# ai4colonoscopy/PraNet-V2

Measured on AMD Instinct MI355X. Metric: images/sec (train fwd+bwd) at 352x352 bs=32/GPU, higher is better.
Workload: dtype bf16; 1 GPU; PraNet-V2 Res2Net50 training step (fwd+4x structure_loss+bwd+clamp+Adam), bs=32/GPU 352x352, random-init, synthetic ellipse masks; global_batch=32, parallelism=dp1, launch=hipGraph replay

## Files before the change

include/pn2.h:

```cpp
#ifndef PN2_H
#define PN2_H
#ifdef __cplusplus
extern "C" {
#endif

#define PN2_F32 0
#define PN2_BF16 1
#define PN2_F32F 2
#define PN2_F32X3 3
#define PN2_CONV_STATS 1
#define PN2_CONV_ACCUM 2
#define PN2_CONV_SPLITK(n) ((n) << 16)
#define PN2_CONV_ROWGATE 8
#define PN2_CONV_AFFINE 16
#define PN2_CONV_RELU 32
#define PN2_CONV_RELU6 64
#define PN2_CONV_BIAS 4

typedef struct pn2_conv_desc {
    int N, H, W;
    int OH, OW;
    int Cin_p, ld_in;
    int Cout, ld_out;
    int KH, KW, stride, pad_h, pad_w, dil_h, dil_w;
// ... 26 lines not shown
int pn2_conv_stat_blocks(int m, int cout, int dtype);
int pn2_conv_gemm(int dtype, const void* in, const void* wp, void* out, float* psum, float* psq, const pn2_conv_desc* d, void* stream);
#define PN2_BNB_STATS 1
#define PN2_BNB_MASK_RAW 2
#define PN2_BNB_MASK_Y 4
#define PN2_BNB_STORE_MASKED 8
int pn2_conv_gemm_gated(int dtype, const void* in, const void* wp, void* out, float* psum, float* psq, const pn2_conv_desc* d, const float* gate, void* stream);
int pn2_conv_gemm_affine(int dtype, const void* in, const void* wp, void* out, const float* scale, const float* shift, const void* res, int ld_res,
                         const pn2_conv_desc* d, void* stream);
typedef struct pn2_bnb_target {
    void* out; int ld_out;
    int mode;
    const void* raw; int ld_raw;
    const void* y; int ld_y;
    const float* par; int ps;
    int split;
    const void* raw2; const float* par2;
    float* p1; float* p2; int ldp;
} pn2_bnb_target;
typedef struct pn2_conv_ep { pn2_bnb_target a, b; const void* pool; int ld_pool; int pad_; pn2_bnb_target c; } pn2_conv_ep;
int pn2_conv_gemm_ep(int dtype, const void* in, const void* wp, void* out, const pn2_conv_desc* d, const pn2_conv_ep* ep, void* stream);
typedef struct pn2_conv_job { const void* in; const void* wp; void* out; float* psum; float* psq; pn2_conv_desc d; int pad_; pn2_conv_ep ep; } pn2_conv_job;
int pn2_conv_gemm_tile(int dtype, const pn2_conv_desc* d);
int pn2_conv_gemm_job_blocks(int dtype, const pn2_conv_job* j, int bm, int bn);
int pn2_conv_gemm_multi(int dtype, int bm, int bn, int ep, const pn2_conv_job* jobs_dev, const int* block_start_dev, int njobs, int total_blocks, void* stream);
int pn2_conv_splitk_reduce(int dtype, const float* ws, int ksplit, int M, int Cout, void* out, int ld_out, const float* bias, float* psum, float* psq,
                           int accumulate, void* stream);
int pn2_conv_wgrad(int dtype, const void* dy, const void* x, float* slab, const pn2_wgrad_desc* d, int nsplit, void* stream);
typedef struct pn2_wgrad_job { const void* dy; const void* x; float* slab; pn2_wgrad_desc d; int nsplit;
    int rot;
} pn2_wgrad_job;
int pn2_conv_wgrad_variant(int dtype, const pn2_wgrad_desc* d);
int pn2_conv_wgrad_blocks(const pn2_wgrad_desc* d, int nsplit);
int pn2_conv_wgrad_multi(int dtype, int variant, const pn2_wgrad_job* jobs_dev, const int* block_start_dev, int njobs, int total_blocks, void* stream);
int pn2_pack_weight(int dtype, const float* w_oihw, void* wp, const pn2_pack_desc* p, void* stream);
int pn2_wgrad_reduce(const float* slab, float* gw_oihw, const pn2_pack_desc* p, int nsplit, int accumulate, void* stream);
int pn2_pack_patch_weight(int dtype, const float* w_oihw, void* wp, int Cout, int Cin, int KH, int KW, int Cin_p, int Rp, int Kp, void* stream);
int pn2_depth_to_space(int dtype, const void* t, int ld_t, void* dx, int ld_dx, int N, int H, int W, int OH, int OW, int S, int C, int accumulate, void* stream);
int pn2_conv_dgrad_small_cin(int dtype, const void* dy, int ld_dy, const float* w_oihw, void* dx, int ld_dx, int N, int H, int W, int OH, int OW,
                             int Cout, int Cin, int KH, int KW, int stride, int pad, int accumulate, void* stream);
typedef struct pn2_pack_job { const float* w; void* wp; pn2_pack_desc d; } pn2_pack_job;
int pn2_pack_blocks(const pn2_pack_desc* p);
int pn2_pack_weights_multi(int dtype, const pn2_pack_job* jobs_dev, const int* block_start_dev, int njobs, int total_blocks, void* stream);
typedef struct pn2_reduce_job { const float* slab; float* gw; pn2_pack_desc d; int nsplit; int accumulate; } pn2_reduce_job;
int pn2_wgrad_reduce_blocks(const pn2_pack_desc* p);
int pn2_wgrad_reduce_multi(const pn2_reduce_job* jobs_dev, const int* block_start_dev, int njobs, int total_blocks, void* stream);

typedef struct pn2_bn_desc {
    int M;
    int Cp;
    int C, gw, gwp;
    float eps, momentum;
    int ldp;
    int tile_rows;
} pn2_bn_desc;
int pn2_bn_finalize(const float* psum, const float* psq, int nblk, const pn2_bn_desc* d, const float* gamma, const float* beta,
                    float* running_mean, float* running_var, float* scale, float* shift, float* mean, float* invstd, void* stream);
int pn2_bn_eval_prepare(const pn2_bn_desc* d, const float* gamma, const float* beta, const float* running_mean, const float* running_var,
                        float* scale, float* shift, void* stream);
typedef struct pn2_bnprep_job { const float* gamma; const float* beta; const float* running_mean; const float* running_var; float* scale; float* shift; pn2_bn_desc d; int pad_; } pn2_bnprep_job;
int pn2_bn_eval_prepare_multi(const pn2_bnprep_job* jobs_dev, const int* block_start_dev, int njobs, int total_blocks, void* stream);
int pn2_affine_act(int dt_in, const void* x, int ld_x, int dt_out, void* y, int ld_y, int M, int Cout,
                   const float* scale, const float* shift, const void* res, int ld_res, int relu, void* stream);
int pn2_affine_act_sum(int dt, const void* x, int ld_x, void* y, int ld_y, int M, int C, const float* scale, const float* shift, int relu,
                       const void* add, int ld_add, void* y2, int ld_y2, void* stream);
int pn2_affine_act_tee(int dt, const void* x, int ld_x, void* y, int ld_y, int M, int C, const float* scale, const float* shift, int relu,
// ... 289 lines not shown
```

pranet-v2_amd/csrc/pn2_conv.hip:

```cpp
#include <cstring>
#include "pn2_common.h"
#include "../../include/pn2.h"

namespace {

constexpr int ROWB = 128;
constexpr int KSUB = ROWB / 64;
constexpr int RS = ROWB;

#ifdef PN2_STAMP
constexpr int PN2_STAMP_SLOTS = 16, PN2_STAMP_BLOCKS = 1 << 16;
__device__ unsigned long long pn2_stamp_buf[PN2_STAMP_BLOCKS * PN2_STAMP_SLOTS];
__device__ __forceinline__ void pn2_stamp(int i) {
    if (threadIdx.x == 0 && blockIdx.y == 0 && blockIdx.x < PN2_STAMP_BLOCKS) pn2_stamp_buf[blockIdx.x * PN2_STAMP_SLOTS + i] = __builtin_amdgcn_s_memtime();
}
__device__ __forceinline__ void pn2_stamp_hw() {
    if (threadIdx.x == 0 && blockIdx.y == 0 && blockIdx.x < PN2_STAMP_BLOCKS) {
        pn2_stamp_buf[blockIdx.x * PN2_STAMP_SLOTS + 10] = __builtin_amdgcn_s_getreg((31 << 11) | 4);
        pn2_stamp_buf[blockIdx.x * PN2_STAMP_SLOTS + 11] = __builtin_amdgcn_s_getreg((31 << 11) | 20);
    }
}
#define PN2_STAMP_AT(i) pn2_stamp(i)
#else
#define PN2_STAMP_AT(i)
// ... 1694 lines not shown
#pragma unroll
                for (int i = 0; i < MT; ++i) {
                    asm volatile("ds_read_b64_tr_b16 %0, %1" : "=v"(a0[i]) : "v"(sb + offA[i] + ks * 32 * RBY));
                    asm volatile("ds_read_b64_tr_b16 %0, %1" : "=v"(a1[i]) : "v"(sb + offA[i] + (ks * 32 + 16) * RBY));
                }
#pragma unroll
                for (int j = 0; j < NT; ++j) {
                    asm volatile("ds_read_b64_tr_b16 %0, %1" : "=v"(b0[j]) : "v"(sb + offB[j] + ks * 32 * RBX));
                    asm volatile("ds_read_b64_tr_b16 %0, %1" : "=v"(b1[j]) : "v"(sb + offB[j] + (ks * 32 + 16) * RBX));
                }
                asm volatile("s_waitcnt lgkmcnt(0)" ::: "memory");
                __builtin_amdgcn_sched_barrier(0);
#pragma unroll
                for (int i = 0; i < MT; ++i)
#pragma unroll
                    for (int j = 0; j < NT; ++j)
                        MMA<bf16_t>::run(acc[i][j], make_uint4(a0[i].x, a0[i].y, a1[i].x, a1[i].y), make_uint4(b0[j].x, b0[j].y, b1[j].x, b1[j].y));
            }
        }
    }
#undef PN2_WISSUE
    float* dst = slab + ((size_t)split * d.Rp + co0) * d.Kp + k0;
#pragma unroll
    for (int i = 0; i < MT; ++i)
#pragma unroll
        for (int j = 0; j < NT; ++j) {
            if (BNK > 128 && k0 + wn * WTN + j * 16 >= d.Kp) continue;
#pragma unroll
            for (int r = 0; r < 4; ++r)
                dst[(size_t)(wm * WTM + i * 16 + g * 4 + r) * d.Kp + wn * WTN + j * 16 + l15] = acc[i][j][r];
        }
}

template <typename T, int BMC, int BNK, int WM, int WN, bool PW>
__global__ __launch_bounds__(256) void conv_wgrad(const T* __restrict__ dy, const T* __restrict__ x, float* __restrict__ slab, pn2_wgrad_desc d, int nsplit) {
    conv_wgrad_body<T, BMC, BNK, WM, WN, PW>(dy, x, slab, d, nsplit, blockIdx.x);
}
template <typename T, int BMC, int BNK, int WM, int WN, bool PW>
__global__ __launch_bounds__(256) void conv_wgrad_tab(const pn2_wgrad_job* __restrict__ jobs, const int* __restrict__ bstart, int njobs) {
    const int total = bstart[njobs];
    for (int b = blockIdx.x; b < total; b += gridDim.x) {
        const int jb = find_job(bstart, njobs, b);
        const pn2_wgrad_job j = jobs[jb];
        const int bl = b - bstart[jb];
        conv_wgrad_body<T, BMC, BNK, WM, WN, PW>((const T*)j.dy, (const T*)j.x, j.slab, j.d, j.nsplit, (bl & ~7) | ((bl - j.rot) & 7));
        __syncthreads();
    }
}
template <int BMC, int WM, int WN, bool PW, int BNK = 128>
__global__ __launch_bounds__(256) void conv_wgrad_dma(const bf16_t* __restrict__ dy, const bf16_t* __restrict__ x, float* __restrict__ slab, pn2_wgrad_desc d, int nsplit) {
    conv_wgrad_dma_body<BMC, WM, WN, PW, BNK>(dy, x, slab, d, nsplit, blockIdx.x);
}
template <int BMC, int WM, int WN, bool PW, int BNK = 128>
__global__ __launch_bounds__(256) void conv_wgrad_dma_tab(const pn2_wgrad_job* __restrict__ jobs, const int* __restrict__ bstart, int njobs) {
    const int total = bstart[njobs];
    for (int b = blockIdx.x; b < total; b += gridDim.x) {
        const int jb = find_job(bstart, njobs, b);
        const pn2_wgrad_job j = jobs[jb];
        const int bl = b - bstart[jb];
        conv_wgrad_dma_body<BMC, WM, WN, PW, BNK>((const bf16_t*)j.dy, (const bf16_t*)j.x, j.slab, j.d, j.nsplit, (bl & ~7) | ((bl - j.rot) & 7));
        __syncthreads();
    }
}

template <int BMC, int WM, int WN, int BNK>
__global__ __launch_bounds__(256, 2) void conv_wgrad_dma_tab_mix(const pn2_wgrad_job* __restrict__ jobs, const int* __restrict__ bstart, int njobs) {
    const int total = bstart[njobs];
    for (int b = blockIdx.x; b < total; b += gridDim.x) {
        const int jb = find_job(bstart, njobs, b);
        const pn2_wgrad_job j = jobs[jb];
        const int bl = b - bstart[jb];
        const int lb = (bl & ~7) | ((bl - j.rot) & 7);
        if (j.d.KH == 1 && j.d.KW == 1 && j.d.stride == 1 && j.d.pad_h == 0 && j.d.pad_w == 0)
            conv_wgrad_dma_body<BMC, WM, WN, true, BNK>((const bf16_t*)j.dy, (const bf16_t*)j.x, j.slab, j.d, j.nsplit, lb);
        else
            conv_wgrad_dma_body<BMC, WM, WN, false, BNK>((const bf16_t*)j.dy, (const bf16_t*)j.x, j.slab, j.d, j.nsplit, lb);
        __syncthreads();
// ... 324 lines not shown
}
template <bool EP>
int gemm_multi_dispatch(int dtype, int bm, int bn, int bits, const pn2_conv_job* jobs, const int* bstart, int njobs, int total, hipStream_t st) {
    const bool ks2 = dtype == PN2_BF16 && (bm & TILE_KS2);
    if (ks2) bm &= 0xff;
    return with_dtype(dtype, [&](auto ty) {
        using T = typename decltype(ty)::type;
        return with_tile(bm, bn, [&](auto tile) {
            using L = decltype(tile);
            constexpr int BM = L::BM, BN = L::BN, WM = L::WM, WN = L::WN;
            if constexpr (sizeof(T) == 2) {
                if constexpr (BN >= 64 && !(BM == 128 && BN == 128)) { if (ks2) return launch_dma_tab_ks2<EP, BM, BN, WM, WN>(jobs, bstart, njobs, total, bits, st); }
                else if (ks2) return -2;
                return launch_dma_tab<EP, BM, BN, WM, WN>(jobs, bstart, njobs, total, bits, st);
            } else if constexpr (BN == 128) return -2;
            else return launch_gather_tab_f32<T, EP, BM, BN, WM, WN>(jobs, bstart, njobs, total, st);
        });
    });
}

constexpr int wg_dma_ring_bytes(int bmc, int bnk) { return 3 * wg_px(bmc) * (bmc * 2 + bnk * 2); }

template <int BMC, int WM, int WN, int BNK = 128>
int launch_wgrad_dma(const void* dy, const void* x, float* slab, const pn2_wgrad_desc& d, int nsplit, hipStream_t st) {
    constexpr int PX = wg_px(BMC), max_b = wg_dma_ring_bytes(BMC, BNK);
    const int M = d.N * d.OH * d.OW;
    const int total_steps = (M + PX - 1) / PX, spb = (total_steps + nsplit - 1) / nsplit;
    const int lds = (spb < 3 ? (spb < 1 ? 1 : spb) : 3) * (max_b / 3);
    const dim3 grid(8 * ((nsplit + 7) / 8) * (d.Rp / BMC) * ((d.Kp + BNK - 1) / BNK));
    if (is_pointwise(d)) return pn2_launch<conv_wgrad_dma<BMC, WM, WN, true, BNK>>(grid, dim3(256), lds, max_b, st, (const bf16_t*)dy, (const bf16_t*)x, slab, d, nsplit);
    return pn2_launch<conv_wgrad_dma<BMC, WM, WN, false, BNK>>(grid, dim3(256), lds, max_b, st, (const bf16_t*)dy, (const bf16_t*)x, slab, d, nsplit);
}

template <typename T>
int wgrad_variant(const pn2_wgrad_desc& d) {
    const int bmc = pn2_wgrad_tile_co(d.Cout_p);
    bool dma = false, wide = false;
    if constexpr (sizeof(T) == 2) {
        dma = d.tune ? d.tune >= 2 : (is_pointwise(d) && d.N * d.OH * d.OW >= 8192);
        if ((size_t)d.N * d.OH * d.OW * d.ld_dy * 2 >= 0x80000000ull || (size_t)d.N * d.H * d.W * d.ld_x * 2 >= 0x80000000ull) dma = false;
        wide = dma && bmc == 128 && d.Kp >= 256 && d.tune == 3;
    }
    if (wide) return 12 + (is_pointwise(d) ? 1 : 0);
    return (dma ? 6 : 0) + (bmc == 128 ? 2 : (bmc == 64 ? 1 : 0)) * 2 + (is_pointwise(d) ? 1 : 0);
}

template <typename T>
inline int wgrad_blocks_t(const pn2_wgrad_desc& d, int nsplit) {
    const int bmc = pn2_wgrad_tile_co(d.Cout_p);
    const int bnk = wgrad_variant<T>(d) >= 12 ? 256 : 128;
    return 8 * ((nsplit + 7) / 8) * (d.Rp / bmc) * ((d.Kp + bnk - 1) / bnk);
}

template <typename T>
int wgrad_dispatch(const void* dy, const void* x, float* slab, const pn2_wgrad_desc& d, int nsplit, hipStream_t st) {
    const int bmc = pn2_wgrad_tile_co(d.Cout_p);
    if (d.Rp % bmc || d.Kp % 128) return -2;
    const int v = wgrad_variant<T>(d);
    return with_wgrad_tile(bmc, [&](auto tile) {
        using L = decltype(tile);
        if constexpr (sizeof(T) == 2) {
            if (v >= 12) return launch_wgrad_dma<128, 2, 2, 256>(dy, x, slab, d, nsplit, st);
            if (v >= 6) return launch_wgrad_dma<L::BM, L::WM, L::WN>(dy, x, slab, d, nsplit, st);
        }
        return launch_wgrad<T, L::BM, L::WM, L::WN>(dy, x, slab, d, nsplit, st);
    });
}

template <typename T, int BMC, int WM, int WN>
int launch_wgrad_tab(bool pw, const pn2_wgrad_job* jobs, const int* bstart, int njobs, int total, hipStream_t st) {
    constexpr int BNK = 128;
    constexpr int lds = 2 * wg_stage_bytes<T>(BMC, BNK), cap = X3<T> ? lds : 0;
    if (pw) return pn2_launch<conv_wgrad_tab<T, BMC, BNK, WM, WN, true>>(dim3(total), dim3(256), lds, cap, st, jobs, bstart, njobs);
    return pn2_launch<conv_wgrad_tab<T, BMC, BNK, WM, WN, false>>(dim3(total), dim3(256), lds, cap, st, jobs, bstart, njobs);
}

template <int BMC, int WM, int WN, int BNK = 128>
int launch_wgrad_dma_tab(bool pw, const pn2_wgrad_job* jobs, const int* bstart, int njobs, int total, hipStream_t st) {
    constexpr int max_b = wg_dma_ring_bytes(BMC, BNK);
    if (pw) return pn2_launch<conv_wgrad_dma_tab<BMC, WM, WN, true, BNK>>(dim3(total), dim3(256), max_b, max_b, st, jobs, bstart, njobs);
    return pn2_launch<conv_wgrad_dma_tab<BMC, WM, WN, false, BNK>>(dim3(total), dim3(256), max_b, max_b, st, jobs, bstart, njobs);
}

template <typename T>
int wgrad_multi_dispatch(int v, const pn2_wgrad_job* jobs, const int* bstart, int njobs, int total, hipStream_t st) {
    const bool pw = v & 1;
    if (v >= 6 && sizeof(T) != 2) return -3;
    return with_wgrad_tile(32 << ((v % 6) >> 1), [&](auto tile) {
        using L = decltype(tile);
        if constexpr (sizeof(T) == 2) {
            constexpr int wide_b = wg_dma_ring_bytes(128, 256);
            if (v == 14) return pn2_launch<conv_wgrad_dma_tab_mix<128, 2, 2, 256>>(dim3(total), dim3(256), wide_b, wide_b, st, jobs, bstart, njobs);
            if (v >= 12) return launch_wgrad_dma_tab<128, 2, 2, 256>(pw, jobs, bstart, njobs, total, st);
            if (v >= 6) return launch_wgrad_dma_tab<L::BM, L::WM, L::WN>(pw, jobs, bstart, njobs, total, st);
        }
        return launch_wgrad_tab<T, L::BM, L::WM, L::WN>(pw, jobs, bstart, njobs, total, st);
    });
}


template <typename T>
__global__ __launch_bounds__(256) void pack_patch_k(const float* __restrict__ w, T* __restrict__ wp, int Cout, int Cin, int KH, int KW, int Cin_p, int Rp, int Kp) {
    const size_t total = (size_t)Rp * Kp;
    for (size_t i = (size_t)blockIdx.x * 256 + threadIdx.x; i < total; i += (size_t)gridDim.x * 256) {
        const int row = (int)(i / Kp), k = (int)(i - (size_t)row * Kp);
        const int tap = row / Cin_p, ci = row - tap * Cin_p;
        float v = 0.f;
// ... 261 lines not shown
    if (!j || !j->in || !j->wp || !j->out || bm < 1 || bn < 1) return -1;
    const pn2_conv_desc& d = j->d;
    if ((d.flags & PN2_CONV_STATS) && (!j->psum || !j->psq)) return -1;
    if ((d.flags & PN2_CONV_BIAS) && !j->psum) return -1;
    if (d.flags & PN2_CONV_AFFINE) {
        const int v_ = dtype == PN2_BF16 ? 8 : 4;
        if (!j->psum || !j->psq || (d.flags & (PN2_CONV_STATS | PN2_CONV_BIAS | PN2_CONV_ACCUM | PN2_CONV_ROWGATE)) || j->ep.a.mode || j->ep.b.mode || j->ep.b.out) return -1;
        if (j->ep.a.y && (d.Cout % v_ || d.ld_out % v_ || j->ep.a.ld_y % v_)) return -2;
    }
    const bool use_ep = (j->ep.a.mode | j->ep.b.mode) != 0 || j->ep.b.out != nullptr;
    const int vec = dtype == PN2_BF16 ? 8 : 4;
    if (use_ep && (d.Cout % vec || d.ld_out % vec || (d.flags & (PN2_CONV_STATS | PN2_CONV_BIAS)))) return -2;
    return ((d.N * d.OH * d.OW + bm - 1) / bm) * ((d.Cout + bn - 1) / bn);
}

int pn2_conv_gemm_multi(int dtype, int bm, int bn, int ep, const pn2_conv_job* jobs_dev, const int* block_start_dev, int njobs, int total_blocks, void* stream) {
    if (!jobs_dev || !block_start_dev || njobs < 1 || total_blocks < 1) return -1;
    return (ep & 1) ? gemm_multi_dispatch<true>(dtype, bm, bn, ep >> 1, jobs_dev, block_start_dev, njobs, total_blocks, (hipStream_t)stream)
                    : gemm_multi_dispatch<false>(dtype, bm, bn, 0, jobs_dev, block_start_dev, njobs, total_blocks, (hipStream_t)stream);
}

int pn2_conv_wgrad(int dtype, const void* dy, const void* x, float* slab, const pn2_wgrad_desc* d, int nsplit, void* stream) {
    if (!dy || !x || !slab || !d || nsplit < 1) return -1;
    if (d->Cin_p % 8 || d->ld_x % 8 || d->ld_dy % 8 || d->Cout_p % 8) return -2;
    if (dtype != PN2_BF16 && d->tune >= 2) return -2;
    return with_dtype(dtype, [&](auto ty) { return wgrad_dispatch<typename decltype(ty)::type>(dy, x, slab, *d, nsplit, (hipStream_t)stream); });
}

int pn2_conv_wgrad_variant(int dtype, const pn2_wgrad_desc* d) {
    if (!d) return -1;
    return with_dtype(dtype, [&](auto ty) { return sizeof(typename decltype(ty)::type) == 2 ? wgrad_variant<bf16_t>(*d) : wgrad_variant<float>(*d); });
}

int pn2_conv_wgrad_blocks(const pn2_wgrad_desc* d, int nsplit) {
    if (!d || nsplit < 1) return -1;
    const int bmc = pn2_wgrad_tile_co(d->Cout_p);
    if (d->Rp % bmc || d->Kp % 128) return -2;
    return wgrad_blocks_t<bf16_t>(*d, nsplit);
}

int pn2_conv_wgrad_multi(int dtype, int variant, const pn2_wgrad_job* jobs_dev, const int* block_start_dev, int njobs, int total_blocks, void* stream) {
    if (!jobs_dev || !block_start_dev || njobs < 1 || total_blocks < 1 || variant < 0 || variant >= 15) return -1;
    return with_dtype(dtype, [&](auto ty) { return wgrad_multi_dispatch<typename decltype(ty)::type>(variant, jobs_dev, block_start_dev, njobs, total_blocks, (hipStream_t)stream); });
}

int pn2_pack_weight(int dtype, const float* w, void* wp, const pn2_pack_desc* p, void* stream) {
    if (!w || !wp || !p) return -1;
    const size_t total = (size_t)p->Rp * p->Kp;
    const int grid = (int)((total + 255) / 256 > 4096 ? 4096 : (total + 255) / 256);
    if (dtype == PN2_BF16) hipLaunchKernelGGL(pack_weight<bf16_t>, dim3(grid), dim3(256), 0, (hipStream_t)stream, w, (bf16_t*)wp, *p);
    else if (dtype == PN2_F32) hipLaunchKernelGGL(pack_weight<float>, dim3(grid), dim3(256), 0, (hipStream_t)stream, w, (float*)wp, *p);
    else return -3;
    PN2_CHECK_LAUNCH();
    return 0;
}

int pn2_pack_blocks(const pn2_pack_desc* p) { return (p && p->KH * p->KW <= 225) ? pack_blocks(*p) : -1; }

int pn2_pack_weights_multi(int dtype, const pn2_pack_job* jobs_dev, const int* block_start_dev, int njobs, int total_blocks, void* stream) {
    if (!jobs_dev || !block_start_dev || njobs < 1 || total_blocks < 1) return -1;
    if (dtype == PN2_BF16) hipLaunchKernelGGL(pack_weight_multi<bf16_t>, dim3(total_blocks), dim3(256), 0, (hipStream_t)stream, jobs_dev, block_start_dev, njobs);
    else if (dtype == PN2_F32) hipLaunchKernelGGL(pack_weight_multi<float>, dim3(total_blocks), dim3(256), 0, (hipStream_t)stream, jobs_dev, block_start_dev, njobs);
    else return -3;
    PN2_CHECK_LAUNCH();
    return 0;
}
// ... 86 lines not shown
```

pranet-v2_amd/pn2/capi.py:

```python
import ctypes as C
import os

_HERE = os.path.dirname(os.path.abspath(__file__))
LIB_PATH = os.environ.get("PN2_LIB") or os.path.join(os.path.dirname(_HERE), "csrc", "libpn2_hip.so")

F32, BF16 = 0, 1
F32F = 2
F32X3 = 3
CONV_STATS, CONV_ACCUM, CONV_BIAS = 1, 2, 4
CONV_AFFINE, CONV_RELU, CONV_RELU6 = 16, 32, 64


class ConvDesc(C.Structure):
    _fields_ = [(n, C.c_int) for n in ("N", "H", "W", "OH", "OW", "Cin_p", "ld_in", "Cout", "ld_out", "KH", "KW", "stride",
                                       "pad_h", "pad_w", "dil_h", "dil_w", "transposed", "Kp", "flags")]


class WgradDesc(C.Structure):
    _fields_ = [(n, C.c_int) for n in ("N", "H", "W", "OH", "OW", "Cin_p", "ld_x", "Cout_p", "ld_dy", "KH", "KW", "stride",
                                       "pad_h", "pad_w", "dil_h", "dil_w", "Rp", "Kp", "tune")]


class PackDesc(C.Structure):
    _fields_ = [(n, C.c_int) for n in ("Cout", "Cin", "KH", "KW", "Cout_p", "gw_out", "gwp_out", "Cin_p", "gw_in", "gwp_in",
# ... 104 lines not shown


class RaggedHeader(C.Structure):
    _fields_ = [(n, C.c_int) for n in ("magic", "N", "blocks0", "blocks1", "max_out", "uniform_out", "desc_off", "bs0_off", "bs1_off", "tab_off", "ntables", "pad_")] + \
               [(n, C.c_longlong) for n in ("bytes", "work_doubles", "src_elems", "out_elems")]


RAGGED_MAX_N = 4096
P, I, LL, FL = C.c_void_p, C.c_int, C.c_longlong, C.c_float

SIGNATURES = {
    "pn2_conv_tile_n": [I],
    "pn2_wgrad_tile_co": [I],
    "pn2_conv_tile_m": [I, I, I],
    "pn2_conv_stat_blocks": [I, I, I],
    "pn2_conv_gemm": [I, P, P, P, P, P, C.POINTER(ConvDesc), P],
    "pn2_conv_gemm_ep": [I, P, P, P, C.POINTER(ConvDesc), C.POINTER(ConvEp), P],
    "pn2_conv_gemm_tile": [I, C.POINTER(ConvDesc)],
    "pn2_conv_gemm_job_blocks": [I, C.POINTER(ConvJob), I, I],
    "pn2_conv_gemm_multi": [I, I, I, I, P, P, I, I, P],
    "pn2_bn_finalize_job_blocks": [C.POINTER(BnFinJob)],
    "pn2_bn_finalize_multi": [P, P, I, I, P],
    "pn2_affine_job_blocks": [I, C.POINTER(AffineJob)],
    "pn2_affine_multi": [I, P, P, I, I, P],
    "pn2_bn_bwd_finalize_job_blocks": [C.POINTER(BnBFinJob)],
    "pn2_bn_bwd_finalize_multi": [P, P, I, I, P],
    "pn2_bn_bwd_apply_job_blocks": [I, C.POINTER(BnApplyJob)],
    "pn2_bn_bwd_apply_multi": [I, P, P, I, I, P],
    "pn2_bn_bwd_reduce_job_blocks": [I, C.POINTER(BnReduceJob)],
    "pn2_bn_bwd_reduce_multi": [I, P, P, I, I, P],
    "pn2_conv_wgrad": [I, P, P, P, C.POINTER(WgradDesc), I, P],
    "pn2_conv_wgrad_variant": [I, C.POINTER(WgradDesc)],
    "pn2_conv_wgrad_blocks": [C.POINTER(WgradDesc), I],
    "pn2_conv_wgrad_multi": [I, I, P, P, I, I, P],
    "pn2_pack_weight": [I, P, P, C.POINTER(PackDesc), P],
    "pn2_conv_dgrad_small_cin": [I, P, I, P, P, I, I, I, I, I, I, I, I, I, I, I, I, I, P],
    "pn2_conv_splitk_reduce": [I, P, I, I, I, P, I, P, P, P, I, P],
    "pn2_pack_patch_weight": [I, P, P, I, I, I, I, I, I, I, P],
    "pn2_depth_to_space": [I, P, I, P, I, I, I, I, I, I, I, I, I, P],
    "pn2_wgrad_reduce": [P, P, C.POINTER(PackDesc), I, I, P],
    "pn2_pack_blocks": [C.POINTER(PackDesc)],
    "pn2_pack_weights_multi": [I, P, P, I, I, P],
    "pn2_wgrad_reduce_blocks": [C.POINTER(PackDesc)],
    "pn2_wgrad_reduce_multi": [P, P, I, I, P],
    "pn2_bn_finalize": [P, P, I, C.POINTER(BnDesc), P, P, P, P, P, P, P, P, P],
    "pn2_bn_eval_prepare": [C.POINTER(BnDesc), P, P, P, P, P, P, P],
    "pn2_bn_eval_prepare_multi": [P, P, I, I, P],
    "pn2_affine_act_sum": [I, P, I, P, I, I, I, P, P, I, P, I, P, I, P],
    "pn2_affine_act_tee": [I, P, I, P, I, I, I, P, P, I, P, I, I, P],
    "pn2_affine_act_dual": [I, P, I, P, P, P, I, P, P, P, I, I, I, I, P],
    "pn2_bn_relu_maxpool_fwd": [I, P, I, P, P, P, I, P, I, I, I, I, I, I, P],
    "pn2_pool_bn_bwd_reduce": [I, P, I, P, P, I, I, I, I, I, I, I, P, P, P, P, P, P, I, P],
    "pn2_pool_bn_bwd_apply": [I, P, I, P, P, I, I, I, I, I, I, I, P, P, P, P, P, P, I, P],
    "pn2_affine_act": [I, P, I, I, P, I, I, I, P, P, P, I, I, P],
    "pn2_bn_bwd_reduce": [I, I, P, I, I, P, I, I, P, I, I, I, P, P, P, P, I, P, P, I, P],
    "pn2_bn_bwd_blocks": [I, I, I],
    "pn2_bn_bwd_finalize": [P, P, I, C.POINTER(BnDesc), P, P, P, P, I, P, P],
    "pn2_bn_bwd_finalize_seg": [C.POINTER(BnSegs), C.POINTER(BnDesc), P, P, P, P, I, P, P],
    "pn2_bn_bwd_apply": [I, I, P, I, I, P, I, I, P, I, I, I, P, P, P, P, I, P, I, I, P, P, I, P],
    "pn2_bn_bwd_apply_dual": [I, P, I, I, I, P, I, P, P, P, P, I, P, I, P, P, P, P, I, P],
    "pn2_maxpool3x3s2_fwd": [I, P, I, P, I, P, I, I, I, I, I, I, P],
    "pn2_maxpool3x3s2_bwd": [I, P, I, P, P, I, I, I, I, I, I, I, P],
    "pn2_avgpool_fwd": [I, P, I, P, I, I, I, I, I, I, I, I, I, I, I, P],
    "pn2_avgpool_bwd": [I, P, I, P, I, I, I, I, I, I, I, I, I, I, I, I, P],
    "pn2_bilinear_fwd": [I, P, I, P, I, I, I, I, I, I, I, I, FL, FL, P],
    "pn2_bilinear_bwd": [I, P, I, P, I, I, I, I, I, I, I, I, FL, FL, I, P],
# ... 98 lines not shown
    "pn2_eval_wfm": [P, P, I, I, P, C.c_double, P, P, P, P],
    "pn2_eval_tail_batch": [P, I, I, I, I, P, I, I, LL, P, P, P],
    "pn2_eval_counts_batch": [P, P, P, I, I, I, LL, P, P, P],
    "pn2_eval_wfm_batch": [P, P, P, I, I, I, LL, P, C.c_double, P, P, P, P],
    "pn2_seg_labels": [P, I, I, I, I, I, I, P, P],
    "pn2_seg_labels_up": [C.POINTER(SegUpMap), I, I, I, I, I, I, P, P],
    "pn2_seg_counts": [P, P, LL, I, P, P],
    "pn2_seg_surface_workspace": [I, I, I, I, C.POINTER(LL)],
    "pn2_seg_surface_hist_len": [I, I, I],
    "pn2_seg_surface_hist": [P, P, I, I, I, I, I, P, P, P, P],
    "pn2_zoom_tables": [I, I, I, P, P, P],
    "pn2_zoom_pole_pow": [I, P],
    "pn2_zoom_workspace": [I, I, I, C.POINTER(LL)],
    "pn2_zoom_prefilter": [P, I, I, I, P, P],
    "pn2_zoom3_gather": [P, I, I, I, I, I, P, P, P, P, P, P, P, P],
    "pn2_zoom0": [I, P, I, I, I, I, I, P, P, P, P, P, P],
    "pn2_rotate0": [I, P, I, I, I, P, P, P],
    "pn2_rot_flip": [I, P, I, I, P, P, P],
    "pn2_ragged_plan_bound": [I, P, C.POINTER(LL)],
    "pn2_ragged_plan": [I, P, I, P, LL],
    "pn2_ragged_prefilter": [P, P, P, P, P],
    "pn2_ragged_zoom3": [P, P, P, P, P, P],
    "pn2_ragged_zoom0": [P, P, P, P, P],
    "pn2_ragged_dice_counts": [P, P, P, P, P, P],
    "pn2_ag_blocks": [I, I, I, I],
    "pn2_ag_psi_rows": [I, I, I],
    "pn2_ag_psi_fwd": [I, P, I, P, P, P, I, P, P, P, I, I, I, P, P, P, P],
    "pn2_ag_apply_fwd": [I, P, I, P, I, P, P, P, P, I, I, I, I, P],
    "pn2_ag_bwd_gate": [I, P, I, P, I, P, P, P, P, P, P, I, I, P, I, I, P, P, P, I, I, I, P],
    "pn2_ag_bwd_sum": [I, P, P, P, P, P, P, P, I, P, P, P, I, P, P, P, I, I, I, P, I, P, P, P],
}
_VALUE_FUNCS = {"pn2_copy_job_blocks", "pn2_conv_gemm_tile", "pn2_conv_gemm_job_blocks", "pn2_bn_finalize_job_blocks", "pn2_affine_job_blocks", "pn2_bn_bwd_finalize_job_blocks",
                "pn2_bn_bwd_apply_job_blocks", "pn2_bn_bwd_reduce_job_blocks", "pn2_dwconv3x3_colsum_blocks", "pn2_resize_ksize", "pn2_input_batch_blocks", "pn2_colsum_job_blocks", "pn2_colsum_finalize_blocks", "pn2_dwconv3x3_wgrad_blocks", "pn2_conv_tile_n", "pn2_wgrad_tile_co", "pn2_conv_stat_blocks", "pn2_conv_tile_m", "pn2_bn_bwd_blocks", "pn2_loss_blocks",
                "pn2_pack_blocks", "pn2_wgrad_reduce_blocks", "pn2_conv_wgrad_variant", "pn2_conv_wgrad_blocks",
                "pn2_dsra_tail_blocks", "pn2_dsra_tail_scratch", "pn2_dsra_tail_fused_ok", "pn2_dsra_tail_fused_scratch", "pn2_ln_slots", "pn2_rows_blocks", "pn2_colsum_unit", "pn2_attn_bwd_blocks", "pn2_attn_long_bwd_blocks", "pn2_mutation_loss_blocks", "pn2_mutation_loss_width", "pn2_dual_loss_width", "pn2_seg_loss_width",
                "pn2_dwconv_blocks", "pn2_ag_blocks", "pn2_ag_psi_rows", "pn2_pairconv_blocks", "pn2_msdc_combine_tile", "pn2_gate_blocks", "pn2_eval_wfm_blocks", "pn2_seg_surface_hist_len"}

_lib = None
WORK = {}


def load():
    global _lib
    if _lib is not None:
        return _lib
    if not os.path.exists(LIB_PATH):
        raise RuntimeError(f"{LIB_PATH} not found: build it with `make -C pranet-v2_amd/csrc` (or __graft_entry__.build()); "
                           "pranet-v2_amd has no CPU / PyTorch fallback path")
    lib = C.CDLL(LIB_PATH)
    for name, args in SIGNATURES.items():
        fn = getattr(lib, name)
        fn.argtypes = args
        fn.restype = C.c_int
    _lib = lib
    return lib


class _Caller:

    def __getattr__(self, name):
        fn = getattr(load(), name)
        if name in _VALUE_FUNCS:
            return fn

        def checked(*a):
            rc = fn(*a)
            if rc != 0:
# ... 7 lines not shown
```

pranet-v2_amd/pn2/ops_conv.py:

```python
import ctypes as C
from functools import partial
from types import SimpleNamespace

import torch

from . import capi
from . import core
from .capi import call, F32, BF16, F32F, F32X3
from .core import (Act, Bnb, KSPLIT_MINK, TUNE_REPS, WGRAD_SLAB_MB, WGRAD_WGS, _LinearAsConv, _job_table, _p, _stream, _thrash, _w4, rup)

KS_UNTUNED = 3 | (1 << 2) | (2 << 4) | 0x40
_MMA_KEY = {F32F: "f32f", F32X3: "f32x3"}

def _relu_code(relu):
    return (2 if relu == 2 else 1) if relu else 0


def _conv_desc(N, H, W, OH, OW, Cin_p, ld_in, Cout, ld_out, k=(1, 1, 1, 0, 0, 1, 1), transposed=0, Kp=0, flags=0):
    d = capi.ConvDesc()
    d.N, d.H, d.W, d.OH, d.OW = N, H, W, OH, OW
    d.Cin_p, d.ld_in, d.Cout, d.ld_out = Cin_p, ld_in, Cout, ld_out
    d.KH, d.KW, d.stride, d.pad_h, d.pad_w, d.dil_h, d.dil_w = k
    d.transposed, d.Kp, d.flags = transposed, Kp, flags
    return d


def _wgrad_desc(N, H, W, OH, OW, Cin_p, ld_x, Cout_p, k, Kp):
    d = capi.WgradDesc()
    d.N, d.H, d.W, d.OH, d.OW = N, H, W, OH, OW
    d.Cin_p, d.ld_x, d.Cout_p, d.ld_dy = Cin_p, ld_x, Cout_p, Cout_p
    d.KH, d.KW, d.stride, d.pad_h, d.pad_w, d.dil_h, d.dil_w = k
    tco = call.pn2_wgrad_tile_co(Cout_p)
    d.Rp, d.Kp = rup(Cout_p, tco), Kp
    return d, tco


def _wgrad_splits(M, wd, tco):
    tiles = (wd.Rp // tco) * (wd.Kp // 128)
    steps = (M + 31) // 32
    return max(1, min(steps // 4 if steps >= 8 else 1, (WGRAD_WGS + tiles - 1) // tiles, (WGRAD_SLAB_MB << 20) // (wd.Rp * wd.Kp * 4) or 1))


def _bn_desc(bn, M, Cp, C_, gw, gwp, ldp=0, tile_rows=0):
    d = capi.BnDesc()
    d.M, d.Cp, d.C, d.gw, d.gwp, d.eps, d.momentum = M, Cp, C_, gw, gwp, bn.eps, (bn.momentum if bn.momentum is not None else 0.1)
    d.ldp, d.tile_rows = ldp, tile_rows
    return d


def _time_candidates(cands, run, admit=None):
    kept, evs = [], []
    for c in cands:
        if admit is None:
            run(c)
        elif not admit(c, kept):
            continue
        kept.append(c)
        per = []
        for _ in range(TUNE_REPS):
            if core.TUNE_COLD:
                _thrash()
            e0, e1 = torch.cuda.Event(enable_timing=True), torch.cuda.Event(enable_timing=True)
            e0.record()
            run(c)
            e1.record()
            per.append((e0, e1))
        evs.append(per)
    torch.cuda.synchronize()
    times = [min(a.elapsed_time(b) for a, b in per) for per in evs]
    return kept[min(range(len(kept)), key=lambda i: times[i])] if kept else None

# ... 508 lines not shown
            else:
                return residual.grad_sink()
        return None, 0

    def _bwd_no_bn(self, s):
        bias, dy = s.bias, s.dy
        if s.bn is not None:
            raise RuntimeError("backward through eval-mode BatchNorm is not supported")
        bias_done = bias is None
        if bias is not None and s.dt_dy == F32 and self.dt != F32 or (bias is not None and s.Cdy != s.Cp):
            gb, gba = self.pgrads.sink(bias)
            call.pn2_bias_grad(_p(dy), s.M, s.Cdy, _p(gb), gba, s.st)
            bias_done = True
        rg, racc = self._bwd_residual_sink(s)
        if s.ymask is None and rg is None and s.dt_dy == self.dt and s.Cdy == s.Cp and dy.stride(2) == s.Cp and dy.is_contiguous():
            s.draw = dy
        else:
            self._bn_bwd_apply(s, None, s.draw, rg, racc)
        return bias_done

    def _bwd_gate(self, s):
        gate, draw, M, Cp, st = s.gate, s.draw, s.M, s.Cp, s.st
        gc_, cacc = gate.grad_sink()
        dc = self.fbuf(M) if cacc else gc_
        dzg = draw if draw is not s.dy else self.alloc((s.N, s.OH, s.OW, Cp), self.tdt)
        call.pn2_ra_gate_post_bwd(self.dt, _p(s.raw), s.raw_ld, gate.ptr, _p(draw), Cp, _p(dzg), Cp, _p(dc), M, Cp, st)
        if cacc:
            call.pn2_copy(F32, _p(dc), 1, F32, _p(gc_), 1, M, 1, 1, st)
        s.draw = dzg

    def _wgrad(self, s, draw, Kp, weights, slab_key):
        x, M, st = s.x, s.M, s.st
        wd, tco = _wgrad_desc(s.N, s.H, s.W, s.OH, s.OW, x.Cp, x.ld, s.Cp, s.k, Kp)
        nsplit = _wgrad_splits(M, wd, tco)
        rds = [self._pack_desc(w, s.x_map, o_map, False) for w, o_map, _off in weights]
        for rd in rds:
            rd.Rp = wd.Rp
        wd.tune, nsplit = self._tune_wgrad(wd, _p(draw), x.ptr, rds[0], nsplit, weights[0][0].shape)
        rq = self.grad_queue
        defer = rq is not None and rq.defer_wgrad
        if defer:
            nsplit = rq.table_splits(nsplit, M, x.Cp + s.Cp, wd, 4 if self.dt == F32 else 2)
        slab = self.fbuf(nsplit, wd.Rp, wd.Kp) if rq is None else rq.slab(slab_key, (nsplit, wd.Rp, wd.Kp), self.dev)
        if defer:
            rq.add_wgrad(self.mma, draw, x.ptr, x.t, slab, wd, nsplit, s.flops)
        else:
            capi.WORK.update(flops=s.flops, tag="", shape=s.shape)
            call.pn2_conv_wgrad(self.mma, _p(draw), x.ptr, _p(slab), C.byref(wd), nsplit, st)
        for (w, _o_map, off), rd in zip(weights, rds):
            gwt, gwa = self.pgrads.sink(w)
            if rq is None:
                call.pn2_wgrad_reduce(_p(slab[:, off:]), _p(gwt), C.byref(rd), nsplit, gwa, st)
            else:
                rq.add_reduce(slab[:, off:], gwt, rd, nsplit, gwa)

    def _dgrad_patch(self, s):
        x, draw, N, OH, OW, KH, KW, Cp, st = s.x, s.draw, s.N, s.OH, s.OW, s.KH, s.KW, s.Cp, s.st
        gx, gxa = x.grad_sink()
        Ct = KH * KW * x.Cp
        Rp2, Kp2 = rup(Ct, 128), rup(Cp, 128)
        wp2 = self.alloc((Rp2, Kp2), self.tdt)
        call.pn2_pack_patch_weight(self.dt, _p(s.w), _p(wp2), s.Cout, s.Cin, KH, KW, x.Cp, Rp2, Kp2, st)
        tpatch = self.empty(N, OH, OW, Ct)
        dd = _conv_desc(N, OH, OW, OH, OW, Cp, Cp, Ct, Ct, Kp=Kp2)
        dd.flags |= self._tune_gemm(dd, _p(draw), wp2, s.M, Ct) << 8
        capi.WORK.update(flops=s.flops, tag=":dgrad", shape=s.shape + " patch")
        call.pn2_conv_gemm(self.mma, _p(draw), _p(wp2), _p(tpatch), C.c_void_p(0), C.c_void_p(0), C.byref(dd), st)
        call.pn2_depth_to_space(self.dt, _p(tpatch), Ct, _p(gx), gx.stride(2), N, s.H, s.W, OH, OW, KH, x.Cp, gxa, st)

    def _dgrad_small_cin(self, s):
        gx, gxa = s.x.grad_sink()
# ... 344 lines not shown
```

Baseline: 2350 images/sec.

## Add tap-reuse wgrad kernel for small-Cout stride-1 convolutions

Adds a specialised bf16 weight-gradient kernel for stride-1, non-dilated KxK convolutions with at most 32 output channels and small Cin. It stages one shared input line window per tap row in LDS and reads all taps from it with transposed LDS reads, instead of gathering an im2col tile per K block. One block covers the whole K dimension, so the split count is recomputed and autotuning is skipped for these layers. The cost is larger dynamic LDS for the table-driven wgrad launch, which can lower occupancy for the other jobs sharing that launch.

```diff
diff --git a/include/pn2.h b/include/pn2.h
--- a/include/pn2.h
+++ b/include/pn2.h
@@ -82,6 +82,7 @@
 } pn2_wgrad_job;
 int pn2_conv_wgrad_variant(int dtype, const pn2_wgrad_desc* d);
 int pn2_conv_wgrad_blocks(const pn2_wgrad_desc* d, int nsplit);
+int pn2_conv_wgrad_taps(int dtype, const pn2_wgrad_desc* d);
 int pn2_conv_wgrad_multi(int dtype, int variant, const pn2_wgrad_job* jobs_dev, const int* block_start_dev, int njobs, int total_blocks, void* stream);
 int pn2_pack_weight(int dtype, const float* w_oihw, void* wp, const pn2_pack_desc* p, void* stream);
 int pn2_wgrad_reduce(const float* slab, float* gw_oihw, const pn2_pack_desc* p, int nsplit, int accumulate, void* stream);
diff --git a/pranet-v2_amd/csrc/pn2_conv.hip b/pranet-v2_amd/csrc/pn2_conv.hip
--- a/pranet-v2_amd/csrc/pn2_conv.hip
+++ b/pranet-v2_amd/csrc/pn2_conv.hip
@@ -1750,17 +1750,176 @@
         }
 }
 
+constexpr int TAPS_NT = 6;
+constexpr int TAPS_NX = 3;
+constexpr int TAPS_LDS = 40 * 1024;
+__host__ __device__ inline int taps_line(int KW, int OW) { return WGP + (KW - 1) * ((WGP - 2) / OW + 2); }
+__host__ __device__ inline int taps_stage_bytes(const pn2_wgrad_desc& d) { return WGP * (32 * 2 + WG<bf16_t>::PAD) + d.KH * taps_line(d.KW, d.OW) * (d.Cin_p * 2 + WG<bf16_t>::PAD); }
+__host__ __device__ inline bool taps_geom_ok(const pn2_wgrad_desc& d) {
+    if (d.stride != 1 || d.dil_h != 1 || d.dil_w != 1 || d.KH * d.KW < 2 || d.KH < 1 || d.KW < 1) return false;
+    if (d.Cout_p > 32 || d.Cout_p % 8 || d.Rp % 32 || d.Cin_p % 16 || d.Cin_p < 16 || d.ld_x % 8 || d.ld_dy % 8) return false;
+    const int ktot = d.KH * d.KW * d.Cin_p;
+    if (ktot > 64 * TAPS_NT || d.Kp > 64 * TAPS_NT || d.Kp < ktot || d.Kp % 16) return false;
+    if (d.N < 1 || d.OH < 1 || d.OW < 1 || d.OH != d.H + 2 * d.pad_h - (d.KH - 1) || d.OW != d.W + 2 * d.pad_w - (d.KW - 1)) return false;
+    if (d.KH * taps_line(d.KW, d.OW) * (d.Cin_p / 8) > 256 * TAPS_NX) return false;
+    return 2 * taps_stage_bytes(d) <= TAPS_LDS;
+}
+
+__device__ __forceinline__ void conv_wgrad_taps_body(const bf16_t* __restrict__ dy, const bf16_t* __restrict__ x, float* __restrict__ slab, const pn2_wgrad_desc& d, int nsplit, int bloc) {
+    constexpr int BMC = 32, MT = 2, NT = TAPS_NT, NX = TAPS_NX;
+    constexpr int RSY = BMC * 2 + WG<bf16_t>::PAD;
+    extern __shared__ __attribute__((aligned(16))) char smem[];
+    const int tid = threadIdx.x, lane = tid & 63, wn = tid >> 6, l15 = lane & 15, g = lane >> 4;
+    const int M = d.N * d.OH * d.OW;
+    const int RSX = d.Cin_p * 2 + WG<bf16_t>::PAD, VPR = d.Cin_p >> 3;
+    const int LINE = taps_line(d.KW, d.OW), OWP = d.OW + d.KW - 1;
+    const int STAGE = WGP * RSY + d.KH * LINE * RSX;
+    const int ntile = d.Rp / BMC;
+    const int xcd = bloc & 7, jx = bloc >> 3;
+    const int split = xcd + 8 * (jx / ntile), co0 = (jx % ntile) * BMC;
+    if (split >= nsplit) return;
+    const int total_steps = (M + WGP - 1) / WGP;
+    const int spb = (total_steps + nsplit - 1) / nsplit;
+    const int s_begin = split * spb;
+    int s_end = s_begin + spb; if (s_end > total_steps) s_end = total_steps;
+
+    const int ycv = tid & 3, yrow = tid >> 2;
+    const bool y_ok = tid < WGP * 4 && co0 + ycv * 8 < d.Cout_p;
+    const int yco = y_ok ? co0 + ycv * 8 : 0;
+    const int nvec = d.KH * LINE * VPR;
+    int xr[NX], xq[NX], xc[NX], xl[NX];
+#pragma unroll
+    for (int i = 0; i < NX; ++i) {
+        const int v = tid + 256 * i, sl = v / VPR;
+        xc[i] = (v - sl * VPR) * 8; xr[i] = sl / LINE; xq[i] = sl - xr[i] * LINE;
+        xl[i] = sl * RSX + xc[i] * 2;
+    }
+    int ox0, oy0, n0;
+    {
+        const int m0 = s_begin < total_steps ? s_begin * WGP : 0, hw = d.OH * d.OW;
+        n0 = m0 / hw; const int rem = m0 - n0 * hw;
+        oy0 = rem / d.OW; ox0 = rem - oy0 * d.OW;
+    }
+    int oxc = ox0;
+
+    uint4 ry, rx[NX];
+    bool ym = false;
+    unsigned xmask = 0;
+    auto gload = [&](int step, bool live) {
+        const int m = step * WGP + yrow;
+        ym = live && y_ok && m < M;
+        ry = *reinterpret_cast<const uint4*>(dy + (size_t)(ym ? m : 0) * d.ld_dy + yco);
+        xmask = 0;
+        const int L0 = d.OW - ox0 + d.KW - 1;
+#pragma unroll
+        for (int i = 0; i < NX; ++i) {
+            if (i * 256 >= nvec) break;
+            int c = xq[i], j = 0, ix;
+            if (c >= L0) { c -= L0; j = 1; while (c >= OWP) { c -= OWP; ++j; } ix = c - d.pad_w; }
+            else ix = ox0 + c - d.pad_w;
+            int oy = oy0 + j, n = n0;
+            while (oy >= d.OH) { oy -= d.OH; ++n; }
+            const int iy = oy + xr[i] - d.pad_h;
+            const bool ok = live && tid + 256 * i < nvec && n < d.N && (unsigned)iy < (unsigned)d.H && (unsigned)ix < (unsigned)d.W;
+            if (ok) xmask |= 1u << i;
+            rx[i] = *reinterpret_cast<const uint4*>(x + (ok ? (size_t)((n * d.H + iy) * d.W + ix) * d.ld_x + xc[i] : 0));
+        }
+        ox0 += WGP;
+        while (ox0 >= d.OW) { ox0 -= d.OW; if (++oy0 >= d.OH) { oy0 = 0; ++n0; } }
+    };
+    auto lstore = [&](int stage) {
+        char* Ys = smem + stage * STAGE;
+        char* Xs = Ys + WGP * RSY;
+        if (tid < WGP * 4) *reinterpret_cast<uint4*>(Ys + yrow * RSY + ycv * 16) = ym ? ry : make_uint4(0, 0, 0, 0);
+#pragma unroll
+        for (int i = 0; i < NX; ++i) {
+            if (i * 256 >= nvec) break;
+            if (tid + 256 * i < nvec) *reinterpret_cast<uint4*>(Xs + xl[i]) = (xmask >> i) & 1u ? rx[i] : make_uint4(0, 0, 0, 0);
+        }
+    };
+
+    const int ncb = (d.KH * d.KW * d.Cin_p) >> 4;
+    int cboff[NT];
+#pragma unroll
+    for (int j = 0; j < NT; ++j) {
+        const int k = (wn + 4 * j) * 16, tap = k / d.Cin_p, r = tap / d.KW;
+        cboff[j] = (r * LINE + (tap - r * d.KW)) * RSX + (k - tap * d.Cin_p + (l15 & 3) * 4) * 2;
+    }
+    f32x4_t acc[MT][NT];
+#pragma unroll
+    for (int i = 0; i < MT; ++i)
+#pragma unroll
+        for (int j = 0; j < NT; ++j) acc[i][j] = f32x4_t{0.f, 0.f, 0.f, 0.f};
+
+    const int p0 = g * 4 + (l15 >> 2);
+    if (s_begin < s_end) {
+        gload(s_begin, true);
+        lstore(0);
+        __syncthreads();
+        for (int step = s_begin; step < s_end; ++step) {
+            const int cur = (step - s_begin) & 1;
+            gload(step + 1, step + 1 < s_end);
+            const char* Ys = smem + cur * STAGE;
+            const char* Xs = Ys + WGP * RSY;
+            int t = oxc + p0, jb = 0;
+            while (t >= d.OW) { t -= d.OW; ++jb; }
+            const int sl0 = (p0 + jb * (d.KW - 1)) * RSX;
+            t += 16;
+            while (t >= d.OW) { t -= d.OW; ++jb; }
+            const int sl1 = (p0 + 16 + jb * (d.KW - 1)) * RSX;
+            uint4 a[MT];
+#pragma unroll
+            for (int i = 0; i < MT; ++i) a[i] = tr_frag_bf16(Ys, RSY, i * 16, lane);
+#pragma unroll
+            for (int j = 0; j < NT; ++j) {
+                if (wn + 4 * j >= ncb) break;
+                const s16x4_t_ v0 = __builtin_amdgcn_ds_read_tr16_b64_v4i16((s16x4_t_ __attribute__((address_space(3)))*)(Xs + cboff[j] + sl0));
+                const s16x4_t_ v1 = __builtin_amdgcn_ds_read_tr16_b64_v4i16((s16x4_t_ __attribute__((address_space(3)))*)(Xs + cboff[j] + sl1));
+                const uint2 lo = __builtin_bit_cast(uint2, v0), hi = __builtin_bit_cast(uint2, v1);
+                const uint4 b = make_uint4(lo.x, lo.y, hi.x, hi.y);
+#pragma unroll
+                for (int i = 0; i < MT; ++i) MMA<bf16_t>::run(acc[i][j], a[i], b);
+            }
+            oxc += WGP;
+            while (oxc >= d.OW) oxc -= d.OW;
+            lstore(cur ^ 1);
+            __syncthreads();
+        }
+    }
+    float* dst = slab + ((size_t)split * d.Rp + co0) * d.Kp;
+#pragma unroll
+    for (int i = 0; i < MT; ++i)
+#pragma unroll
+        for (int j = 0; j < NT; ++j) {
+            const int col = (wn + 4 * j) * 16;
+            if (col >= d.Kp) break;
+#pragma unroll
+            for (int r = 0; r < 4; ++r) dst[(size_t)(i * 16 + g * 4 + r) * d.Kp + col + l15] = acc[i][j][r];
+        }
+}
+
+__global__ __launch_bounds__(256) void conv_wgrad_taps(const bf16_t* __restrict__ dy, const bf16_t* __restrict__ x, float* __restrict__ slab, pn2_wgrad_desc d, int nsplit) {
+    conv_wgrad_taps_body(dy, x, slab, d, nsplit, blockIdx.x);
+}
 template <typename T, int BMC, int BNK, int WM, int WN, bool PW>
 __global__ __launch_bounds__(256) void conv_wgrad(const T* __restrict__ dy, const T* __restrict__ x, float* __restrict__ slab, pn2_wgrad_desc d, int nsplit) {
     conv_wgrad_body<T, BMC, BNK, WM, WN, PW>(dy, x, slab, d, nsplit, blockIdx.x);
 }
 template <typename T, int BMC, int BNK, int WM, int WN, bool PW>
-__global__ __launch_bounds__(256) void conv_wgrad_tab(const pn2_wgrad_job* __restrict__ jobs, const int* __restrict__ bstart, int njobs) {
+__global__ __launch_bounds__(256) void conv_wgrad_tab(const pn2_wgrad_job* __restrict__ jobs, const int* __restrict__ bstart, int njobs, int lds) {
     const int total = bstart[njobs];
     for (int b = blockIdx.x; b < total; b += gridDim.x) {
         const int jb = find_job(bstart, njobs, b);
         const pn2_wgrad_job j = jobs[jb];
         const int bl = b - bstart[jb];
+        if constexpr (sizeof(T) == 2 && !X3<T> && BMC == 32 && !PW) {
+            if (j.d.tune == 4 && taps_geom_ok(j.d)) {
+                if (2 * taps_stage_bytes(j.d) <= lds)
+                    conv_wgrad_taps_body((const bf16_t*)j.dy, (const bf16_t*)j.x, j.slab, j.d, j.nsplit, (bl & ~7) | ((bl - j.rot) & 7));
+                __syncthreads();
+                continue;
+            }
+        }
         conv_wgrad_body<T, BMC, BNK, WM, WN, PW>((const T*)j.dy, (const T*)j.x, j.slab, j.d, j.nsplit, (bl & ~7) | ((bl - j.rot) & 7));
         __syncthreads();
     }
@@ -2151,12 +2310,21 @@
     return pn2_launch<conv_wgrad_dma<BMC, WM, WN, false, BNK>>(grid, dim3(256), lds, max_b, st, (const bf16_t*)dy, (const bf16_t*)x, slab, d, nsplit);
 }
 
+inline bool wgrad_taps_on() { const char* e = getenv("PN2_WGRAD_TAPS"); return !(e && e[0] == '0'); }
+template <typename T>
+inline bool wgrad_taps_ok(const pn2_wgrad_desc& d) { return std::is_same<T, bf16_t>::value && taps_geom_ok(d) && wgrad_taps_on(); }
+
+int launch_wgrad_taps(const void* dy, const void* x, float* slab, const pn2_wgrad_desc& d, int nsplit, hipStream_t st) {
+    const dim3 grid(8 * ((nsplit + 7) / 8) * (d.Rp / 32));
+    return pn2_launch<conv_wgrad_taps>(grid, dim3(256), 2 * taps_stage_bytes(d), TAPS_LDS, st, (const bf16_t*)dy, (const bf16_t*)x, slab, d, nsplit);
+}
+
 template <typename T>
 int wgrad_variant(const pn2_wgrad_desc& d) {
     const int bmc = pn2_wgrad_tile_co(d.Cout_p);
     bool dma = false, wide = false;
     if constexpr (sizeof(T) == 2) {
-        dma = d.tune ? d.tune >= 2 : (is_pointwise(d) && d.N * d.OH * d.OW >= 8192);
+        dma = d.tune ? (d.tune >= 2 && d.tune != 4) : (is_pointwise(d) && d.N * d.OH * d.OW >= 8192);
         if ((size_t)d.N * d.OH * d.OW * d.ld_dy * 2 >= 0x80000000ull || (size_t)d.N * d.H * d.W * d.ld_x * 2 >= 0x80000000ull) dma = false;
         wide = dma && bmc == 128 && d.Kp >= 256 && d.tune == 3;
     }
@@ -2167,6 +2335,7 @@
 template <typename T>
 inline int wgrad_blocks_t(const pn2_wgrad_desc& d, int nsplit) {
     const int bmc = pn2_wgrad_tile_co(d.Cout_p);
+    if (sizeof(T) == 2 && d.tune == 4 && taps_geom_ok(d)) return 8 * ((nsplit + 7) / 8) * (d.Rp / bmc);
     const int bnk = wgrad_variant<T>(d) >= 12 ? 256 : 128;
     return 8 * ((nsplit + 7) / 8) * (d.Rp / bmc) * ((d.Kp + bnk - 1) / bnk);
 }
@@ -2175,6 +2344,7 @@
 int wgrad_dispatch(const void* dy, const void* x, float* slab, const pn2_wgrad_desc& d, int nsplit, hipStream_t st) {
     const int bmc = pn2_wgrad_tile_co(d.Cout_p);
     if (d.Rp % bmc || d.Kp % 128) return -2;
+    if (wgrad_taps_ok<T>(d)) return launch_wgrad_taps(dy, x, slab, d, nsplit, st);
     const int v = wgrad_variant<T>(d);
     return with_wgrad_tile(bmc, [&](auto tile) {
         using L = decltype(tile);
@@ -2189,9 +2359,10 @@
 template <typename T, int BMC, int WM, int WN>
 int launch_wgrad_tab(bool pw, const pn2_wgrad_job* jobs, const int* bstart, int njobs, int total, hipStream_t st) {
     constexpr int BNK = 128;
-    constexpr int lds = 2 * wg_stage_bytes<T>(BMC, BNK), cap = X3<T> ? lds : 0;
-    if (pw) return pn2_launch<conv_wgrad_tab<T, BMC, BNK, WM, WN, true>>(dim3(total), dim3(256), lds, cap, st, jobs, bstart, njobs);
-    return pn2_launch<conv_wgrad_tab<T, BMC, BNK, WM, WN, false>>(dim3(total), dim3(256), lds, cap, st, jobs, bstart, njobs);
+    constexpr int own = 2 * wg_stage_bytes<T>(BMC, BNK), cap = X3<T> ? own : 0;
+    const int lds = (sizeof(T) == 2 && BMC == 32 && !pw && own < TAPS_LDS && wgrad_taps_on()) ? TAPS_LDS : own;
+    if (pw) return pn2_launch<conv_wgrad_tab<T, BMC, BNK, WM, WN, true>>(dim3(total), dim3(256), lds, cap, st, jobs, bstart, njobs, lds);
+    return pn2_launch<conv_wgrad_tab<T, BMC, BNK, WM, WN, false>>(dim3(total), dim3(256), lds, cap, st, jobs, bstart, njobs, lds);
 }
 
 template <int BMC, int WM, int WN, int BNK = 128>
@@ -2519,6 +2690,11 @@
     return with_dtype(dtype, [&](auto ty) { return sizeof(typename decltype(ty)::type) == 2 ? wgrad_variant<bf16_t>(*d) : wgrad_variant<float>(*d); });
 }
 
+int pn2_conv_wgrad_taps(int dtype, const pn2_wgrad_desc* d) {
+    if (!d) return -1;
+    return with_dtype(dtype, [&](auto ty) { return wgrad_taps_ok<typename decltype(ty)::type>(*d) ? 1 : 0; });
+}
+
 int pn2_conv_wgrad_blocks(const pn2_wgrad_desc* d, int nsplit) {
     if (!d || nsplit < 1) return -1;
     const int bmc = pn2_wgrad_tile_co(d->Cout_p);
diff --git a/pranet-v2_amd/pn2/capi.py b/pranet-v2_amd/pn2/capi.py
--- a/pranet-v2_amd/pn2/capi.py
+++ b/pranet-v2_amd/pn2/capi.py
@@ -160,6 +160,7 @@
     "pn2_conv_wgrad": [I, P, P, P, C.POINTER(WgradDesc), I, P],
     "pn2_conv_wgrad_variant": [I, C.POINTER(WgradDesc)],
     "pn2_conv_wgrad_blocks": [C.POINTER(WgradDesc), I],
+    "pn2_conv_wgrad_taps": [I, C.POINTER(WgradDesc)],
     "pn2_conv_wgrad_multi": [I, I, P, P, I, I, P],
     "pn2_pack_weight": [I, P, P, C.POINTER(PackDesc), P],
     "pn2_conv_dgrad_small_cin": [I, P, I, P, P, I, I, I, I, I, I, I, I, I, I, I, I, I, P],
@@ -324,7 +325,7 @@
 }
 _VALUE_FUNCS = {"pn2_copy_job_blocks", "pn2_conv_gemm_tile", "pn2_conv_gemm_job_blocks", "pn2_bn_finalize_job_blocks", "pn2_affine_job_blocks", "pn2_bn_bwd_finalize_job_blocks",
                 "pn2_bn_bwd_apply_job_blocks", "pn2_bn_bwd_reduce_job_blocks", "pn2_dwconv3x3_colsum_blocks", "pn2_resize_ksize", "pn2_input_batch_blocks", "pn2_colsum_job_blocks", "pn2_colsum_finalize_blocks", "pn2_dwconv3x3_wgrad_blocks", "pn2_conv_tile_n", "pn2_wgrad_tile_co", "pn2_conv_stat_blocks", "pn2_conv_tile_m", "pn2_bn_bwd_blocks", "pn2_loss_blocks",
-                "pn2_pack_blocks", "pn2_wgrad_reduce_blocks", "pn2_conv_wgrad_variant", "pn2_conv_wgrad_blocks",
+                "pn2_pack_blocks", "pn2_wgrad_reduce_blocks", "pn2_conv_wgrad_variant", "pn2_conv_wgrad_blocks", "pn2_conv_wgrad_taps",
                 "pn2_dsra_tail_blocks", "pn2_dsra_tail_scratch", "pn2_dsra_tail_fused_ok", "pn2_dsra_tail_fused_scratch", "pn2_ln_slots", "pn2_rows_blocks", "pn2_colsum_unit", "pn2_attn_bwd_blocks", "pn2_attn_long_bwd_blocks", "pn2_mutation_loss_blocks", "pn2_mutation_loss_width", "pn2_dual_loss_width", "pn2_seg_loss_width",
                 "pn2_dwconv_blocks", "pn2_ag_blocks", "pn2_ag_psi_rows", "pn2_pairconv_blocks", "pn2_msdc_combine_tile", "pn2_gate_blocks", "pn2_eval_wfm_blocks", "pn2_seg_surface_hist_len"}
 
diff --git a/pranet-v2_amd/pn2/ops_conv.py b/pranet-v2_amd/pn2/ops_conv.py
--- a/pranet-v2_amd/pn2/ops_conv.py
+++ b/pranet-v2_amd/pn2/ops_conv.py
@@ -35,8 +35,8 @@
     return d, tco
 
 
-def _wgrad_splits(M, wd, tco):
-    tiles = (wd.Rp // tco) * (wd.Kp // 128)
+def _wgrad_splits(M, wd, tco, taps=False):
+    tiles = (wd.Rp // tco) * (1 if taps else wd.Kp // 128)
     steps = (M + 31) // 32
     return max(1, min(steps // 4 if steps >= 8 else 1, (WGRAD_WGS + tiles - 1) // tiles, (WGRAD_SLAB_MB << 20) // (wd.Rp * wd.Kp * 4) or 1))
 
@@ -611,11 +611,15 @@
     def _wgrad(self, s, draw, Kp, weights, slab_key):
         x, M, st = s.x, s.M, s.st
         wd, tco = _wgrad_desc(s.N, s.H, s.W, s.OH, s.OW, x.Cp, x.ld, s.Cp, s.k, Kp)
-        nsplit = _wgrad_splits(M, wd, tco)
+        taps = call.pn2_conv_wgrad_taps(self.mma, C.byref(wd)) == 1
+        nsplit = _wgrad_splits(M, wd, tco, taps)
         rds = [self._pack_desc(w, s.x_map, o_map, False) for w, o_map, _off in weights]
         for rd in rds:
             rd.Rp = wd.Rp
-        wd.tune, nsplit = self._tune_wgrad(wd, _p(draw), x.ptr, rds[0], nsplit, weights[0][0].shape)
+        if taps:
+            wd.tune = 4
+        else:
+            wd.tune, nsplit = self._tune_wgrad(wd, _p(draw), x.ptr, rds[0], nsplit, weights[0][0].shape)
         rq = self.grad_queue
         defer = rq is not None and rq.defer_wgrad
         if defer:
```

New measurement: 2359 images/sec, median of 6. About the same (+0.4%).
